# ESMWG/NoahMP

Measured on AMD Instinct MI355X. Metric: column-steps/sec, higher is better.
Workload: dtype f32

## Files before the change

### noahmp_amd/csrc/nmp_dev_column.hpp

```cpp
#pragma once
#ifndef __HIPCC_RTC__
#include <string.h>
#endif
#include "nmp_dev_sflx.hpp"
#include "nmp_dev_glacier.hpp"

namespace nmp {

struct KArgs {
  noahmp_step_args a;
  Ctx c;
  int ni, nka;
  int nti, ntj;
  int k1;
  int kp_lo, kp_hi;
  int yearlen;
  unsigned long long* err;
  int* counts;
  unsigned long long err_base;
  long t_offset;
  long t_first, t_count;
  long r_land, r_ice, r_skip;
};

constexpr int LAY_SLOTS = 4 * NL + 5 * NSOIL + 3 * NSNOW;

template <int STRIDE>
NMP_DEV Lay<LArr<STRIDE>> make_lay(float* base) {
  Lay<LArr<STRIDE>> y;
  int o = 0;
  y.stc.p = base + o * STRIDE; o += NL;
  y.zsnso.p = base + o * STRIDE; o += NL;
  y.dzsnso.p = base + o * STRIDE; o += NL;
  y.imelt.p = base + o * STRIDE; o += NL;
  y.smc.p = base + (o - L(1)) * STRIDE; o += NSOIL;
  y.sh2o.p = base + (o - L(1)) * STRIDE; o += NSOIL;
  y.sice.p = base + (o - L(1)) * STRIDE; o += NSOIL;
  y.smceq.p = base + (o - L(1)) * STRIDE; o += NSOIL;
  y.btrani.p = base + (o - L(1)) * STRIDE; o += NSOIL;
  y.snice.p = base + o * STRIDE; o += NSNOW;
  y.snliq.p = base + o * STRIDE; o += NSNOW;
  y.ficeold.p = base + o * STRIDE; o += NSNOW;
  return y;
}

#ifdef NMP_WIDE_INDEX
typedef size_t nmp_ij_t;
#define G2(f) k.a.f[ij]
#define G3(f, lev, nk) k.a.f[((size_t)jj * (nk) + (lev)) * k.ni + ii]
#else
typedef uint32_t nmp_ij_t;
template <class T> NMP_DEV T& at32(T* base, uint32_t idx) {
  const uint32_t o = idx * (uint32_t)sizeof(T);
  return *(T*)((char*)base + (size_t)o);
}
#define G2(f) nmp::at32(k.a.f, ij)
#define G3(f, lev, nk) nmp::at32(k.a.f, ((uint32_t)jj * (uint32_t)(nk) + (uint32_t)(lev)) * (uint32_t)k.ni + (uint32_t)ii)
#endif


NMP_DEV bool column_index(const KArgs& k, long t, int& ii, int& jj, nmp_ij_t& ij) {
  if (t >= (long)k.nti * k.ntj) return false;
  const int tj = (int)(t / k.nti), ti = (int)(t - (long)tj * k.nti);
  ii = k.a.its - k.a.ims + ti;
  jj = k.a.jts - k.a.jms + tj;
  ij = (nmp_ij_t)jj * (nmp_ij_t)k.ni + (nmp_ij_t)ii;
  return true;
}

NMP_DEV int column_classify_values(const KArgs& k, float xland, float xice, int ivg, int ii, int jj, nmp_ij_t ij) {
  int ice = (xice >= k.a.xice_thres) ? 1 : ((ivg == k.a.isice) ? -1 : 0);
  const bool water = (xland - 1.5f) >= 0.f;
  if (k.a.itimestep == 1) {
    if (water) {
      G2(smstav) = 1.0f; G2(smstot) = 1.0f;
      for (int l = 0; l < NSOIL; l++) { G3(smois, l, NSOIL) = 1.0f; G3(tslb, l, NSOIL) = 273.16f; }
    } else if (xice == 1.f) {
      G2(smstav) = 1.0f; G2(smstot) = 1.0f;
      for (int l = 0; l < NSOIL; l++) G3(smois, l, NSOIL) = 1.0f;
    }
  }
  if (water) return 2;
  if (ice == 1) {
    for (int l = 0; l < NSOIL; l++) G3(sh2o, l, NSOIL) = 1.0f;
    G2(xlaixy) = 0.01f;
    return 2;
  }
  return (ice == -1) ? 1 : 0;
}

NMP_DEV int column_classify(const KArgs& k, long t, int& ii, int& jj, nmp_ij_t& ij) {
  if (!column_index(k, t, ii, jj, ij)) return 3;
  const float xland = G2(xland), xice = G2(xice);
  const int ivg = G2(ivgtyp);
  return column_classify_values(k, xland, xice, ivg, ii, jj, ij);
}

NMP_DEV void scatter_energy_outputs(const KArgs& k, const Col& s, nmp_ij_t ij) {
  G2(tsk) = s.trad; G2(hfx) = s.fsh; G2(grdflx) = s.ssoil;
  if (s.albedo > -999) G2(albedo) = s.albedo;
  G2(snowc) = s.fsno; G2(emiss) = s.emissi;
  G2(tgxy) = s.tg; G2(eahxy) = s.eah; G2(tahxy) = s.tah; G2(cmxy) = s.cm; G2(chxy) = s.ch;
  G2(alboldxy) = s.albold; G2(taussxy) = s.tauss; G2(sneqvoxy) = s.sneqvo;
  G2(t2mvxy) = s.t2mv; G2(t2mbxy) = s.t2mb; G2(q2mvxy) = s.q2v / (1.0f - s.q2v);
  G2(tradxy) = s.trad; G2(fvegxy) = s.fveg; G2(fsaxy) = s.fsa; G2(firaxy) = s.fira;
  G2(aparxy) = s.apar; G2(psnxy) = s.psn; G2(savxy) = s.sav; G2(sagxy) = s.sag;
  G2(rssunxy) = s.rssun; G2(rsshaxy) = s.rssha; G2(bgapxy) = s.bgap; G2(wgapxy) = s.wgap;
  G2(tgvxy) = s.tgv; G2(tgbxy) = s.tgb; G2(chvxy) = s.chv; G2(chbxy) = s.chb;
  G2(ircxy) = s.irc; G2(irgxy) = s.irg; G2(shcxy) = s.shc; G2(shgxy) = s.shg; G2(evgxy) = s.evg;
  G2(ghvxy) = s.ghv; G2(irbxy) = s.irb; G2(shbxy) = s.shb; G2(evbxy) = s.evb; G2(ghbxy) = s.ghb;
  G2(trxy) = s.tr; G2(evcxy) = s.evc; G2(chleafxy) = s.chleaf; G2(chucxy) = s.chuc;
  G2(chv2xy) = s.chv2; G2(chb2xy) = s.chb2;
}

NMP_DEV void gather_water_state(const KArgs& k, Col& s, nmp_ij_t ij) {
  s.wslake = G2(wslakexy); s.zwt = G2(zwtxy); s.wt = G2(wtxy);
  s.lfmass = G2(lfmassxy); s.rtmass = G2(rtmassxy); s.stmass = G2(stmassxy); s.wood = G2(woodxy);
  s.stblcp = G2(stblcpxy); s.fastcp = G2(fastcpxy);
  s.smcwtd = G2(smcwtdxy);
  s.acc_sfcrunoff = G2(sfcrunoff); s.acc_udrunoff = G2(udrunoff); s.acc_acsnow = G2(acsnow); s.acc_acsnom = G2(acsnom);
  s.acc_rech = G2(rechxy); s.acc_deeprech = G2(deeprechxy);
}

template <int STRIDE, int MODE = 0, bool EARLY = false, class Runner>
NMP_DEV int column_step(const KArgs& k, int cls, int ii, int jj, nmp_ij_t ij, float* base, Runner& runner, int* cls_out = nullptr) {
  Lay<LArr<STRIDE>> y = make_lay<STRIDE>(base);
  Col s = {};
  Parm P = {};
  bool live = (cls == 0);
  int failed = 0;
  int soiltyp_w = 1;
  NMP_TIC0();
  float c_xland = 0.f, c_xice = 0.f;
  int c_ivg = 0;
  if (EARLY) { c_xland = G2(xland); c_xice = G2(xice); c_ivg = G2(ivgtyp); }
  if (EARLY || cls <= 1) {
  int vegtyp = EARLY ? c_ivg : G2(ivgtyp), soiltyp = G2(isltyp);
  const float xice_in = EARLY ? c_xice : G2(xice);
  s.lat = G2(xlatin);
  s.cosz = G2(coszin);
  const float dz8w_in = G3(dz8w, k.k1, k.nka), vegfra_in = G2(vegfra), vegmax_in = G2(vegmax);
  s.tbot = G2(tmn);
  s.sfctmp = G3(t3d, k.k1, k.nka);
  const float qv_in = G3(qv3d, k.k1, k.nka);
  s.uu = G3(u_phy, k.k1, k.nka); s.vv = G3(v_phy, k.k1, k.nka);
  s.soldn = G2(swdown); s.lwdn = G2(glw);
  const float p8w_hi = G3(p8w3d, k.kp_hi, k.nka), p8w_lo = G3(p8w3d, k.kp_lo, k.nka);
  s.psfc = G3(p8w3d, k.k1, k.nka);
  const float rainbl_in = G2(rainbl);
  int isnow_in = G2(isnowxy);
  float smc_in[NSOIL], sh2o_in[NSOIL], tslb_in[NSOIL], smceq_in[NSOIL], tsno_in[3], snice_in[3], snliq_in[3], zsnso_in[NL];
#pragma unroll
  for (int l = 1; l <= NSOIL; l++) {
    smc_in[l - 1] = G3(smois, l - 1, NSOIL); sh2o_in[l - 1] = G3(sh2o, l - 1, NSOIL);
    tslb_in[l - 1] = G3(tslb, l - 1, NSOIL); smceq_in[l - 1] = G3(smoiseq, l - 1, NSOIL);
  }
#pragma unroll
  for (int l = -2; l <= 0; l++) {
    snice_in[l + 2] = G3(snicexy, l + 2, 3); snliq_in[l + 2] = G3(snliqxy, l + 2, 3); tsno_in[l + 2] = G3(tsnoxy, l + 2, 3);
  }
#pragma unroll
  for (int l = -2; l <= NSOIL; l++) zsnso_in[L(l)] = G3(zsnsoxy, l + 2, NSOIL + 3);
  s.sneqv = G2(snow); s.snowh = G2(snowh); s.qsfc = G2(qsfc);
  s.tv = G2(tvxy); s.tg = G2(tgxy); s.canliq = G2(canliqxy); s.canice = G2(canicexy);
  s.eah = G2(eahxy); s.tah = G2(tahxy); s.cm = G2(cmxy); s.ch = G2(chxy); s.fwet = G2(fwetxy);
  s.sneqvo = G2(sneqvoxy); s.albold = G2(alboldxy); s.qsnow = G2(qsnowxy);
  s.lai = G2(xlaixy); s.sai = G2(xsaixy);
  s.tauss = G2(taussxy); s.wa = G2(waxy);
  if (EARLY) {
    cls = column_classify_values(k, c_xland, c_xice, c_ivg, ii, jj, ij);
    if (cls_out) *cls_out = cls;
    if (cls != MODE - 1) return 0;
    live = (cls == 0);
  }
  s.ist = 1; s.isc = 4; s.ice = (cls == 1) ? -1 : 0;
  s.yearlen = k.yearlen; s.julian = k.a.julian;
  if (isnow_in < -NSNOW || isnow_in > 0) raise(s, NOAHMP_ERR_ISNOW_RANGE);
  s.isnow = isnow_in < -NSNOW ? -NSNOW : (isnow_in > 0 ? 0 : isnow_in);
  NMP_ASSUME(s.isnow >= -NSNOW && s.isnow <= 0);
  if (soiltyp == 14 && xice_in == 0.f) soiltyp = 7;
  if (vegtyp == k.a.isurban || vegtyp == 31 || vegtyp == 32 || vegtyp == 33) vegtyp = k.a.isurban;
  NMP_TIC(0);
  redprm(k.c, s, P, vegtyp, soiltyp);
  soiltyp_w = soiltyp;
  NMP_TIC(1);
  s.zlvl = 0.5f * dz8w_in;
  s.shdfac = div_rc(vegfra_in, NMP_RCC(100.f));
  s.shdmax = div_rc(vegmax_in, NMP_RCC(100.f));
  s.q2 = qv_in / (1.0f + qv_in);
  s.sfcprs = (p8w_hi + p8w_lo) * 0.5f;
  s.prcp = div_rc(rainbl_in, k.c.u.dt);
#pragma unroll
  for (int l = 1; l <= NSOIL; l++) {
    y.smc[L(l)] = smc_in[l - 1]; y.sh2o[L(l)] = sh2o_in[l - 1];
    y.stc[L(l)] = tslb_in[l - 1]; y.smceq[L(l)] = smceq_in[l - 1];
    y.sice[L(l)] = 0.f; y.btrani[L(l)] = 0.f;
  }
#pragma unroll
  for (int l = -2; l <= 0; l++) {
    y.stc[L(l)] = tsno_in[l + 2]; y.snice[L(l)] = snice_in[l + 2]; y.snliq[L(l)] = snliq_in[l + 2];
    y.ficeold[L(l)] = (l > s.isnow) ? snice_in[l + 2] / (snice_in[l + 2] + snliq_in[l + 2]) : 0.f;
  }
#pragma unroll
  for (int l = -2; l <= NSOIL; l++) { y.zsnso[L(l)] = zsnso_in[L(l)]; y.dzsnso[L(l)] = 0.f; y.imelt[L(l)] = 0.f; }
  s.rech = 0.f; s.deeprech = 0.f;
  s.co2air = 395.e-06f * s.sfcprs;
  s.o2air = 0.209f * s.sfcprs;
  s.foln = 1.0f;
  if (vegtyp == 25 || vegtyp == 26 || vegtyp == 27) { s.shdfac = 0.0f; s.lai = 0.0f; }
  s.vegtyp = (vegtyp >= 1 && vegtyp <= k.c.ts.lucats) ? vegtyp : 1;
  if (s.err) { failed = s.err; live = false; }
  }

  float qfx_out = 0.f, lh_out = 0.f;
  if constexpr (MODE != 1)
  if (cls == 1 && !failed) {
    s.tbot = nmp_min(s.tbot, 263.15f);
    glacier(k.c, s, y);
    if (s.err) failed = s.err;
    else {
      gather_water_state(k, s, ij);
      glacier_fill_undefined(s);
      qfx_out = s.edir; lh_out = s.fgev;
      scatter_energy_outputs(k, s, ij);
    }
  }
  if constexpr (MODE != 2) {
    float beg_wb = 0.f;
    bool water_inputs = false;
    auto prefetch_water = [&]() {
      gather_water_state(k, s, ij);
      redprm_water(k.c, P, soiltyp_w, s.vegtyp);
      water_inputs = true;
    };
    sflx_energy(k.c, P, s, y, beg_wb, live, runner, prefetch_water);
    if (live) {
      if (s.err) failed = s.err;
      else {
        lh_out = s.fcev + s.fgev + s.fctr;
        scatter_energy_outputs(k, s, ij);
        if (!water_inputs) prefetch_water();
        NMP_TIC(11);
        sflx_water(k.c, P, s, y, beg_wb);
        if (s.err) failed = s.err;
        qfx_out = s.ecan + s.edir + s.etran;
      }
    }
  }
  if (cls > 1 || failed) return failed;
  G2(qfx) = qfx_out; G2(lh) = lh_out;
  G2(smstav) = 0.0f; G2(smstot) = 0.0f;
  G2(sfcrunoff) = s.acc_sfcrunoff + s.runsrf * k.a.dt;
  G2(udrunoff) = s.acc_udrunoff + s.runsub * k.a.dt;
#pragma unroll
  for (int l = 1; l <= NSOIL; l++) {
    G3(smois, l - 1, NSOIL) = y.smc[L(l)]; G3(sh2o, l - 1, NSOIL) = y.sh2o[L(l)];
    G3(tslb, l - 1, NSOIL) = y.stc[L(l)];
  }
  G2(snow) = s.sneqv; G2(snowh) = s.snowh;
  G2(canwat) = s.canliq + s.canice;
  G2(acsnow) = s.acc_acsnow + s.prcp * s.fpice;
  G2(acsnom) = s.acc_acsnom + s.qsnbot * k.a.dt + s.ponding + s.ponding1 + s.ponding2;
  G2(qsfc) = s.qsfc;
  G2(isnowxy) = s.isnow; G2(tvxy) = s.tv; G2(canliqxy) = s.canliq; G2(canicexy) = s.canice;
  G2(fwetxy) = s.fwet; G2(qsnowxy) = s.qsnow;
  G2(wslakexy) = s.wslake; G2(zwtxy) = s.zwt; G2(waxy) = s.wa; G2(wtxy) = s.wt;
#pragma unroll
  for (int l = -2; l <= 0; l++) {
    G3(tsnoxy, l + 2, 3) = y.stc[L(l)]; G3(snicexy, l + 2, 3) = y.snice[L(l)];
    G3(snliqxy, l + 2, 3) = y.snliq[L(l)];
  }
#pragma unroll
  for (int l = -2; l <= NSOIL; l++) G3(zsnsoxy, l + 2, NSOIL + 3) = y.zsnso[L(l)];
  G2(lfmassxy) = s.lfmass; G2(rtmassxy) = s.rtmass; G2(stmassxy) = s.stmass; G2(woodxy) = s.wood;
  G2(stblcpxy) = s.stblcp; G2(fastcpxy) = s.fastcp; G2(xlaixy) = s.lai; G2(xsaixy) = s.sai;
  G2(q2mbxy) = s.q2b / (1.0f - s.q2b);
  G2(neexy) = s.nee; G2(gppxy) = s.gpp; G2(nppxy) = s.npp;
  G2(runsfxy) = s.runsrf; G2(runsbxy) = s.runsub; G2(ecanxy) = s.ecan;
  G2(edirxy) = s.edir; G2(etranxy) = s.etran;
  G2(rechxy) = s.acc_rech + s.rech * 1.E3f;
  G2(deeprechxy) = s.acc_deeprech + s.deeprech;
  G2(smcwtdxy) = s.smcwtd;
  NMP_TIC(15);
  return 0;
}

}
```

### noahmp_amd/csrc/nmp_kernel.hpp

```cpp
#pragma once
#ifndef __HIPCC_RTC__
#include <hip/hip_runtime.h>
#endif
#include "nmp_dev_column.hpp"
#ifndef __HIPCC_RTC__
#include "nmp_engine_host.hpp"
#else
namespace nmp_host { constexpr int kCountSlots = 256, kCountStride = 16; }
#endif

namespace {
using namespace nmp;

#ifndef NMP_WAVES_PER_EU
#define NMP_WAVES_PER_EU 2
#endif
#ifndef NMP_FIXED_BLOCK
#define NMP_FIXED_BLOCK 64
#endif

template <int BLOCK, bool USE_LDS, int MODE>
__device__ __forceinline__ void column_kernel_body(const KArgs& k, float* lds, const long blk, const long first, const long count) {
  constexpr int STRIDE = USE_LDS ? BLOCK : 1;
  float priv[(USE_LDS || MODE == 3) ? 1 : LAY_SLOTS];
  float* base = USE_LDS ? (lds + threadIdx.x) : priv;

  if (MODE != 3) libm::libm_stage_tables();
  const long tl = blk * BLOCK + threadIdx.x;
  const long t = first + tl;
  int ii = 0, jj = 0;
  nmp_ij_t ij = 0;
  int cls = 3, err = 0;
  if (MODE == 1 || MODE == 2) {
    if (tl < count && column_index(k, t, ii, jj, ij)) {
      SimpleLoop runner;
      err = column_step<STRIDE, MODE, true>(k, -1, ii, jj, ij, base, runner, &cls);
    }
  } else {
    cls = (MODE != 0 && tl >= count) ? 3 : column_classify(k, t, ii, jj, ij);
  }
  {
    unsigned long long m0 = __ballot(cls == 0), m1 = __ballot(cls == 1), m2 = __ballot(cls == 2);
    if ((threadIdx.x & 63) == 0) {
      int* cnt = k.counts + (blockIdx.x % nmp_host::kCountSlots) * nmp_host::kCountStride;
      if (m0) atomicAdd(&cnt[0], __popcll(m0));
      if (m1) atomicAdd(&cnt[1], __popcll(m1));
      if (m2) atomicAdd(&cnt[2], __popcll(m2));
    }
  }
  if (MODE != 0 && cls != 3 && cls != MODE - 1) {
    atomicMin(k.err, k.err_base | ((unsigned long long)(t + k.t_offset + 1) << 8) | (unsigned)NOAHMP_ERR_CLASS_RANGE);
    return;
  }
  if (MODE == 1 || MODE == 2) {
    if (err) atomicMin(k.err, k.err_base | ((unsigned long long)(t + k.t_offset + 1) << 8) | (unsigned)err);
    return;
  }
  if (cls > 1 || MODE == 3) return;
  SimpleLoop runner;
  err = column_step<STRIDE, (MODE == 3 ? 0 : MODE)>(k, cls, ii, jj, ij, base, runner);
  if (err) atomicMin(k.err, k.err_base | ((unsigned long long)(t + k.t_offset + 1) << 8) | (unsigned)err);
}

template <int BLOCK, bool USE_LDS, int MODE = 0>
__global__ void __launch_bounds__(BLOCK, NMP_WAVES_PER_EU) noahmp_column_kernel(const KArgs k) {
  __shared__ float lds[(USE_LDS && MODE != 3) ? LAY_SLOTS * BLOCK : 1];
  column_kernel_body<BLOCK, USE_LDS, MODE>(k, lds, (long)blockIdx.x, k.t_first, k.t_count);
}

template <int BLOCK>
__global__ void __launch_bounds__(BLOCK, NMP_WAVES_PER_EU) noahmp_ranges_kernel(const KArgs k) {
  __shared__ float lds[LAY_SLOTS * BLOCK];
  const long nb_ice = (k.r_ice + BLOCK - 1) / BLOCK, nb_land = (k.r_land + BLOCK - 1) / BLOCK;
  const long b = (long)blockIdx.x;
  if (b < nb_ice) column_kernel_body<BLOCK, true, 2>(k, lds, b, k.r_land, k.r_ice);
  else if (b < nb_ice + nb_land) column_kernel_body<BLOCK, true, 1>(k, lds, b - nb_ice, 0L, k.r_land);
  else column_kernel_body<BLOCK, true, 3>(k, lds, b - nb_ice - nb_land, k.r_land + k.r_ice, k.r_skip);
}

}
```

### noahmp_amd/csrc/nmp_libm.hpp

```cpp
#pragma once
#ifndef __HIPCC_RTC__
#include <hip/hip_runtime.h>
#include <stdint.h>
#include <string.h>
#endif

namespace nmp {
namespace libm {

#ifndef NMP_LIBM_DEV
#define NMP_LIBM_DEV __host__ __device__ __forceinline__
#endif
#ifndef NMP_LIBM_FN
#define NMP_LIBM_FN NMP_LIBM_DEV
#endif
#ifndef NMP_LIBM_FN_POW
#define NMP_LIBM_FN_POW NMP_LIBM_FN
#endif

#if defined(__HIP_DEVICE_COMPILE__)
#define NMP_LIBM_TABLE static __device__ const
#else
#define NMP_LIBM_TABLE static const
#endif
#include "nmp_libm_tables.inc"
#ifndef NMP_LIBM_LDS
#define NMP_LIBM_LDS 1
#endif
#if defined(__HIP_DEVICE_COMPILE__) && NMP_LIBM_LDS
static __shared__ uint64_t sExp2fTab[32];
static __shared__ double sLogfTab[32];
static __shared__ double sPowfLog2Tab[32];
#define NMP_T_EXP2F sExp2fTab
#define NMP_T_LOGF sLogfTab
#define NMP_T_POWLOG2 sPowfLog2Tab
__device__ __forceinline__ void libm_stage_tables() {
  const int t = threadIdx.y * blockDim.x + threadIdx.x;
  if (t < 32) {
    sExp2fTab[t] = kExp2fTab[t];
    sLogfTab[t] = kLogfTab[t];
    sPowfLog2Tab[t] = kPowfLog2Tab[t];
  }
  __syncthreads();
}
#else
#define NMP_T_EXP2F kExp2fTab
#define NMP_T_LOGF kLogfTab
#define NMP_T_POWLOG2 kPowfLog2Tab
__host__ __device__ __forceinline__ void libm_stage_tables() {}
#endif

NMP_LIBM_DEV double mad(double a, double b, double c) { return __builtin_fma(a, b, c); }

NMP_LIBM_DEV uint32_t asuint(float f) { uint32_t u; memcpy(&u, &f, 4); return u; }
NMP_LIBM_DEV float asfloat(uint32_t u) { float f; memcpy(&f, &u, 4); return f; }
NMP_LIBM_DEV uint64_t asuint64(double f) { uint64_t u; memcpy(&u, &f, 8); return u; }
NMP_LIBM_DEV double asdouble(uint64_t u) { double f; memcpy(&f, &u, 8); return f; }
NMP_LIBM_DEV uint64_t exp2_tab_scale_(uint64_t tab, uint64_t k) {
#if defined(__HIP_DEVICE_COMPILE__)
  if (!__builtin_constant_p(k)) {
    typedef uint32_t u32x2 __attribute__((ext_vector_type(2)));
    u32x2 w = __builtin_bit_cast(u32x2, tab);
    w.y += (uint32_t)k << (52 - 5 - 32);
    return __builtin_bit_cast(uint64_t, w);
  }
#endif
  return tab + (k << (52 - 5));
}

NMP_LIBM_DEV bool expf_is_special_(float x) { return !(__builtin_fabsf(x) <= 88.0f); }
NMP_LIBM_DEV float expf_special_(float x, float res) {
  res = (x > 0x1.62e42ep6f) ? asfloat(0x7f800000u) : res;
  res = (x < -0x1.9fe368p6f) ? 0.0f : res;
  res = (x != x) ? x + x : res;
  return res;
}
NMP_LIBM_FN float expf_(float x) {
  const double xd = (double)x;
  double z = kExpfInvLn2Scaled * xd;
  double kd = z + kExp2fShift;
  const uint64_t ki = asuint64(kd);
  kd -= kExp2fShift;
  const double r = mad(kExpfInvLn2Scaled, xd, -kd);
  const uint64_t t = exp2_tab_scale_(NMP_T_EXP2F[ki % 32], ki);
  const double s = asdouble(t);
  z = mad(kExp2fPolyScaled[0], r, kExp2fPolyScaled[1]);
  const double r2 = r * r;
  double y = mad(kExp2fPolyScaled[2], r, 1.0);
  y = mad(z, r2, y);
  y = y * s;
  float res = (float)y;
  if (__builtin_expect(expf_is_special_(x), 0)) res = expf_special_(x, res);
  return res;
}

NMP_LIBM_DEV float expf_k_(float x) {
  const double xd = (double)x;
  double z = kExpfInvLn2Scaled * xd;
  double kd = z + kExp2fShift;
  const uint64_t ki = asuint64(kd);
  kd -= kExp2fShift;
  const double r = mad(kExpfInvLn2Scaled, xd, -kd);
  const uint64_t t = exp2_tab_scale_(kExp2fTab[ki % 32], ki);
  const double s = asdouble(t);
  z = mad(kExp2fPolyScaled[0], r, kExp2fPolyScaled[1]);
  const double r2 = r * r;
  double y = mad(kExp2fPolyScaled[2], r, 1.0);
  y = mad(z, r2, y);
  y = y * s;
  float res = (float)y;
  res = (x > 0x1.62e42ep6f) ? asfloat(0x7f800000u) : res;
  res = (x < -0x1.9fe368p6f) ? 0.0f : res;
  res = (x != x) ? x + x : res;
  return res;
}

NMP_LIBM_DEV bool logf_is_special_(uint32_t ix) { return ix - 0x00800000u >= 0x7f800000u - 0x00800000u; }
NMP_LIBM_DEV uint32_t logf_normalise_(float x, uint32_t ix) {
  return (ix - 1u < 0x007fffffu) ? asuint(x * 0x1p23f) - (23u << 23) : ix;
}
NMP_LIBM_DEV float logf_fix_special_(uint32_t ix0, float x, float res) {
  res = (ix0 == 0x7f800000u) ? x : res;
  res = ((ix0 & 0x80000000u) || ix0 * 2 > 0xff000000u) ? asfloat(0x7fc00000u) : res;
  res = (ix0 * 2 == 0) ? -asfloat(0x7f800000u) : res;
  return res;
}
NMP_LIBM_FN float logf_(float x) {
  const uint32_t ix0 = asuint(x);
  uint32_t ix = ix0;
  if (__builtin_expect(logf_is_special_(ix0), 0)) ix = logf_normalise_(x, ix0);
  const uint32_t tmp = ix - 0x3f330000u;
  const int i = (tmp >> (23 - 4)) % 16;
  const int k = (int32_t)tmp >> 23;
  const uint32_t iz = ix - (tmp & 0xff800000u);
  const double invc = NMP_T_LOGF[2 * i], logc = NMP_T_LOGF[2 * i + 1];
  const double z = (double)asfloat(iz);
  const double r = mad(z, invc, -1.0);
  const double y0 = mad((double)k, kLogfLn2, logc);
  const double r2 = r * r;
  double y = mad(kLogfPoly[1], r, kLogfPoly[2]);
  y = mad(kLogfPoly[0], r2, y);
  y = mad(y, r2, y0 + r);
  float res = (float)y;
  if (__builtin_expect(logf_is_special_(ix0), 0)) res = logf_fix_special_(ix0, x, res);
  return res;
}

#if defined(__HIP_DEVICE_COMPILE__)
#define NMP_LIBM_PIN() __builtin_amdgcn_sched_barrier(0)
#else
#define NMP_LIBM_PIN() ((void)0)
#endif
template <int N>
NMP_LIBM_DEV void logfN_(const float* x, float* out) {
  uint32_t ix0[N], ixn[N], iz[N]; int k[N]; double invc[N], logc[N];
  bool special = false;
#pragma unroll
  for (int n = 0; n < N; n++) {
    ix0[n] = asuint(x[n]);
    ixn[n] = ix0[n];
    special = special || logf_is_special_(ix0[n]);
  }
  if (__builtin_expect(special, 0)) {
#pragma unroll
    for (int n = 0; n < N; n++) ixn[n] = logf_normalise_(x[n], ix0[n]);
  }
#pragma unroll
  for (int n = 0; n < N; n++) {
    const uint32_t ix = ixn[n];
    const uint32_t tmp = ix - 0x3f330000u;
    const int i = (tmp >> (23 - 4)) % 16;
    k[n] = (int32_t)tmp >> 23;
    iz[n] = ix - (tmp & 0xff800000u);
    invc[n] = NMP_T_LOGF[2 * i]; logc[n] = NMP_T_LOGF[2 * i + 1];
  }
  NMP_LIBM_PIN();
#pragma unroll
  for (int n = 0; n < N; n++) {
    const double z = (double)asfloat(iz[n]);
    const double r = mad(z, invc[n], -1.0);
    const double y0 = mad((double)k[n], kLogfLn2, logc[n]);
    const double r2 = r * r;
    double y = mad(kLogfPoly[1], r, kLogfPoly[2]);
    y = mad(kLogfPoly[0], r2, y);
    y = mad(y, r2, y0 + r);
    out[n] = (float)y;
  }
  if (__builtin_expect(special, 0)) {
#pragma unroll
    for (int n = 0; n < N; n++) out[n] = logf_fix_special_(ix0[n], x[n], out[n]);
  }
}
template <int N>
NMP_LIBM_DEV void expfN_(const float* x, float* out) {
  double r[N]; uint64_t t[N];
#pragma unroll
  for (int n = 0; n < N; n++) {
    const double xd = (double)x[n];
    const double z = kExpfInvLn2Scaled * xd;
    double kd = z + kExp2fShift;
    const uint64_t ki = asuint64(kd);
    kd -= kExp2fShift;
// ... 592 lines not shown
```

### noahmp_amd/csrc/noahmp_engine.hip

```cpp
#include <hip/hip_runtime.h>
#include <stdio.h>
#include <stdlib.h>
#include <string.h>
#include <string>
#include <vector>
#include "noahmp_hip.h"
#define NMP_WIDE_INDEX 1
#include "nmp_kernel.hpp"
#include "nmp_stage.hpp"

using namespace nmp;

namespace {

struct FieldDesc { const char* name; size_t off; int kind; int lev; int io; };
#define FD(n, kind, lev, io) {#n, offsetof(noahmp_step_args, n), kind, lev, io}
const FieldDesc kFields[] = {
#include "nmp_fields.inc"
};
constexpr int kNumFields = sizeof(kFields) / sizeof(kFields[0]);

}

namespace nmp_host {
// ... 100 lines not shown
  if (rc) return rc;
  if (!bytes) return 0;
  if (kind == 2) { HIPCHK(hipMemcpy(dst, src, bytes, hipMemcpyDeviceToDevice)); return 0; }
  rc = kind == 0 ? nmp_host::copy_h2d(dst, src, bytes, g.own_stream) : nmp_host::copy_d2h(dst, src, bytes, g.own_stream);
  if (rc) return rc;
  HIPCHK(hipStreamSynchronize(g.own_stream));
  return 0;
}
void noahmp_hip_free(void* p) { if (p) hipFree(p); }

static void drop_host_regs();

int noahmp_hip_debug_live_host_registrations(void) {
  int n = 0;
  for (auto& kv : g.host_regs) n += kv.second.state == 1;
  return n;
}

int noahmp_hip_set_tables(const noahmp_tables* t) {
  int rc = ensure_init();
  if (rc) return rc;
  drop_host_regs();
  g.out_mirror_valid = false;
  static nmp::TablesDev img;
  img.t = *t;
  nmp::derive_tables(img.t, img.d);
  if (!g.d_tables) HIPCHK(hipMalloc((void**)&g.d_tables, sizeof(nmp::TablesDev)));
  HIPCHK(hipMemcpy(g.d_tables, &img, sizeof(nmp::TablesDev), hipMemcpyHostToDevice));
  nmp::tab_scalars_pack(nmp::tab_scalars(img.t), g.ts_i, g.ts_f);
  g.have_tables = true;
  return 0;
}

static void note_fetch(int rc) {
  if (rc > 0) {
    g.deferred_code = rc;
    g.last_error = std::string("a fatal column of the previous (deferred) step is pending: ") + noahmp_hip_error_string(rc);
  }
}

int noahmp_hip_set_option(const char* key, int value) {
  int prev = -1;
  if (!strcmp(key, "block")) { prev = g.block; if (value == 64 || value == 128 || value == 256) g.block = value; }
  else if (!strcmp(key, "lds")) { prev = g.use_lds; g.use_lds = value ? 1 : 0; }
  else if (!strcmp(key, "host_chunks")) {
    prev = g.host_chunks_auto ? -2 : g.host_chunks;
    if (value == -1 || value == -2) g.host_chunks_auto = true;
    else if (value >= 0 && value <= 32) { g.host_chunks = value; g.host_chunks_auto = false; }
  }
  else if (!strcmp(key, "pin_host_arrays")) {
    prev = g.pin_host_arrays;
    if (value == 0 || value == 1) {
      g.pin_host_arrays = value;
      if (!value) drop_host_regs();
    }
  }
  else if (!strcmp(key, "trust_out_mirror")) {
    prev = g.trust_out_mirror;
    if (value == 0 || value == 1) { g.trust_out_mirror = value; g.out_mirror_valid = false; }
  }
  else if (!strcmp(key, "jit_option_kernels")) { prev = g.jit_kernels; if (value == 0 || value == 1) g.jit_kernels = value; }
  else if (!strcmp(key, "jit_compile_only")) { prev = g.jit_compile_only; if (value == 0 || value == 1) g.jit_compile_only = value; }
  else if (!strcmp(key, "fixed_option_kernels")) { prev = g.fixed_kernels; if (value == 0 || value == 1) g.fixed_kernels = value; }
  else if (!strcmp(key, "sorted_land_columns")) { prev = (int)g.sorted_land; g.sorted_land = value; }
  else if (!strcmp(key, "sorted_glacier_columns")) { prev = (int)g.sorted_glacier; g.sorted_glacier = value; }
  else if (!strcmp(key, "resident_state")) {
    prev = g.resident_state;
    if (value == 0 || value == 1) {
      if (!value && (g.resident_dirty || g.deferred_pending)) note_fetch(noahmp_hip_fetch(nullptr));
      g.resident_state = value; g.resident_valid = false;
    }
  }
  else if (!strcmp(key, "resident_sorted")) {
    prev = g.resident_sorted;
    if (value == 0 || value == 1) {
      if (value != g.resident_sorted && (g.resident_dirty || g.deferred_pending)) note_fetch(noahmp_hip_fetch(nullptr));
      if (value != g.resident_sorted) { g.resident_sorted = value; g.sorted_ok = false; g.resident_valid = false; }
    }
  }
  else if (!strcmp(key, "lazy_download")) {
    prev = g.lazy_download;
    if (value == 0 || value == 1) {
      if (!value && (g.resident_dirty || g.deferred_pending)) note_fetch(noahmp_hip_fetch(nullptr));
      g.lazy_download = value;
    }
  }
  else if (!strcmp(key, "overlap_class_kernels")) prev = 1;
  else if (!strcmp(key, "static_inputs")) {
    prev = g.static_inputs;
    if ((value == 0 || value == 1) && value != g.static_inputs) {
      if (g.resident_dirty || g.deferred_pending) note_fetch(noahmp_hip_fetch(nullptr));
      g.static_inputs = value; g.sorted_ok = false; g.sorted_newer = false; g.resident_valid = false;
    }
  }
  else if (!strcmp(key, "deferred_status")) {
    prev = g.deferred_status;
    if (value == 0 || value == 1) {
      if (g.deferred_pending || g.resident_dirty) note_fetch(noahmp_hip_fetch(nullptr));
      g.deferred_status = value; g.resident_valid = false;
    }
  }
  else if (!strcmp(key, "record_cost")) {
#ifdef NMP_COST_RECORD
    prev = g.record_cost;
    if (value == 0 || value == 1) { g.record_cost = value; if (!value) g.cost_fresh = false; }
#endif
  }
  else if (!strcmp(key, "exact_libm")) prev = NMP_EXACT_LIBM;
  return prev;
}

}

static void fill_kargs(KArgs& k, const noahmp_step_args* a) {
  memset(&k, 0, sizeof(k));
  k.a = *a;
  k.ni = a->ime - a->ims + 1;
  k.nka = a->kme - a->kms + 1;
  k.nti = a->ite - a->its + 1;
  k.ntj = a->jte - a->jts + 1;
  k.k1 = 1 - a->kms;
  k.kp_lo = a->kts - a->kms;
  k.kp_hi = a->kts + 1 - a->kms;
  k.yearlen = 365;
  if (a->yr % 4 == 0) { k.yearlen = 366; if (a->yr % 100 == 0) { k.yearlen = 365; if (a->yr % 400 == 0) k.yearlen = 366; } }
  k.c.T = g.d_tables;
  k.c.D = derived_of(g.d_tables);
  k.c.O = Opt{a->idveg, a->iopt_crs, a->iopt_btr, a->iopt_run, a->iopt_sfc, a->iopt_frz, a->iopt_inf,
              a->iopt_rad, a->iopt_alb, a->iopt_snf, a->iopt_tbot, a->iopt_stc};
  k.c.dt = a->dt;
  k.c.isurban = a->isurban;
  k.c.ts = tab_scalars_unpack(g.ts_i, g.ts_f);
  k.c.zsoil[L(1)] = -a->dzs[0];
  for (int l = 2; l <= NOAHMP_NSOIL; l++) k.c.zsoil[L(l)] = -a->dzs[l - 1] + k.c.zsoil[L(l - 1)];
  ctx_fill_uniform(k.c);
  k.err = g.d_err;
  k.counts = g.d_counts;
  k.a.dzs = nullptr;
}

#ifndef NMP_NO_FIXED_KERNELS
struct FixedKernel { int dveg, run; void (*launch)(const nmp_host::LaunchDesc&, int, hipStream_t, hipEvent_t, hipEvent_t); };
static const FixedKernel kFixed[] = {{1, 1, nmp_host::launch_fixed_d1_r1}, {3, 1, nmp_host::launch_fixed_d3_r1},
                                     {3, 5, nmp_host::launch_fixed_d3_r5}, {4, 1, nmp_host::launch_fixed_d4_r1},
                                     {4, 3, nmp_host::launch_fixed_d4_r3}};
#endif
static int fixed_level(const KArgs& k) {
#ifdef NMP_NO_FIXED_KERNELS
  return 0;
#else
  const Opt& o = k.c.O;
  if (!g.fixed_kernels) return 0;
  if (noahmp_hip_index_width(k.ni, k.a.jme - k.a.jms + 1, k.nka) != 32) return 0;
  if (!(o.crs == 1 && o.btr == 1 && o.sfc == 1 && o.frz == 1 && o.inf == 1 && o.rad == 3 && o.alb == 2 &&
        o.snf == 1 && o.tbot == 2 && o.stc == 1)) return g.jit_kernels ? -1 : 0;
  for (int n = 0; n < (int)(sizeof(kFixed) / sizeof(kFixed[0])); n++)
    if (kFixed[n].dveg == o.dveg && kFixed[n].run == o.run) return n + 1;
  return g.jit_kernels ? -1 : 0;
#endif
}

static bool launch_fixed(const KArgs& k, int level, int mode, hipStream_t s, hipEvent_t ev0 = nullptr, hipEvent_t ev1 = nullptr) {
#ifdef NMP_NO_FIXED_KERNELS
  return false;
#else
  nmp_host::LaunchDesc d;
  memset(&d, 0, sizeof(d));
  d.a = k.a; d.tables = k.c.T; d.dt = k.c.dt; d.isurban = k.c.isurban;
  for (int n = 0; n < 6; n++) d.ts_i[n] = g.ts_i[n];
  for (int n = 0; n < 15; n++) d.ts_f[n] = g.ts_f[n];
  for (int l = 0; l < NL; l++) d.zsoil[l] = k.c.zsoil[l];
  d.ni = k.ni; d.nka = k.nka; d.nti = k.nti; d.ntj = k.ntj; d.k1 = k.k1; d.kp_lo = k.kp_lo; d.kp_hi = k.kp_hi; d.yearlen = k.yearlen;
  d.err = k.err; d.counts = k.counts; d.err_base = k.err_base; d.t_offset = k.t_offset; d.t_first = k.t_first; d.t_count = k.t_count;
  d.cost = k.c.cost;
  d.r_land = k.r_land; d.r_ice = k.r_ice; d.r_skip = k.r_skip;
  if (level > 0) { kFixed[level - 1].launch(d, mode, s, ev0, ev1); return true; }
  const Opt& o = k.c.O;
  const int opts[12] = {o.dveg, o.crs, o.btr, o.run, o.sfc, o.frz, o.inf, o.rad, o.alb, o.snf, o.tbot, o.stc};
  return nmp_host::launch_jit(opts, d, mode, s, ev0, ev1);
#endif
}

static void launch_ranges(KArgs k, long n_land, long n_ice, long n_skip, hipStream_t s, hipEvent_t ev0, hipEvent_t ev1) {
  constexpr long B = NMP_FIXED_BLOCK;
  k.r_land = n_land; k.r_ice = n_ice; k.r_skip = n_skip;
  k.t_first = 0; k.t_count = n_land + n_ice + n_skip;
  const long nb_ice = (n_ice + B - 1) / B, nb = nb_ice + (n_land + B - 1) / B + (n_skip + B - 1) / B;
  if (nb <= 0) return;
  if (k.c.cost) k.c.cost -= 2 * nb_ice * B;
  const int fx = fixed_level(k);
  if (fx && launch_fixed(k, fx, 4, s, ev0, ev1)) return;
  hipExtLaunchKernelGGL((noahmp_ranges_kernel<NMP_FIXED_BLOCK>), dim3((unsigned)nb), dim3(NMP_FIXED_BLOCK), 0, s, ev0, ev1, 0, k);
}

static void launch_any(const KArgs& k_in, hipStream_t s, bool class_ranges = false, hipEvent_t* ev = nullptr) {
  KArgs k = k_in;
  const long ncol = (long)k.nti * k.ntj;
  g.last_launch_kind = 0;
  if (ncol <= 0) { g.last_launch_kind = -1; return; }
  k.c.cost = nullptr;
  if (g.record_cost && class_ranges && k.t_offset == 0) {
    if (nmp_host::ensure_bytes((void**)&g.d_cost, &g.d_cost_bytes, (size_t)ncol * 2) == 0) {
      if (g.cost_cols != ncol) (void)hipMemsetAsync(g.d_cost, 0, (size_t)ncol * 2, s);
      k.c.cost = g.d_cost; g.cost_cols = ncol; g.cost_fresh = true;
    }
  }
  if (class_ranges && g.sorted_land >= 0 && g.sorted_glacier >= 0 && g.sorted_land + g.sorted_glacier <= ncol && k.t_offset == 0 &&
      g.block == 256 && g.use_lds) {
    g.last_launch_kind = 1;
    launch_ranges(k, g.sorted_land, g.sorted_glacier, ncol - g.sorted_land - g.sorted_glacier, s, ev ? ev[0] : nullptr, ev ? ev[1] : nullptr);
    return;
  }
  if (ev) hipEventRecord(ev[0], s);
  struct EndEvent { hipEvent_t* e; hipStream_t s; ~EndEvent() { if (e) hipEventRecord(e[1], s); } } at_end{ev, s};
  if (g.block == 256 && g.use_lds) {
    const int fx = fixed_level(k);
    if (fx) { k.t_first = 0; k.t_count = ncol; if (launch_fixed(k, fx, 0, s)) return; }
  }
  if (g.block == 256) launch<256>(k, ncol, g.use_lds, s);
  else if (g.block == 128) launch<128>(k, ncol, g.use_lds, s);
  else launch<64>(k, ncol, g.use_lds, s);
}

static int check_step_args(const noahmp_step_args* a, noahmp_status* st) {
  if (!g.have_tables) { g.last_error = "noahmp_hip_set_tables() has not been called"; return -102; }
  if (a->nsoil != NOAHMP_NSOIL) { if (st) st->code = NOAHMP_ERR_NSOIL_UNSUPPORTED; return NOAHMP_ERR_NSOIL_UNSUPPORTED; }
  if (a->iopt_sfc != 1 && a->iopt_sfc != 2) {
    if (st) st->code = NOAHMP_ERR_OPT_SFC_UNSUPPORTED;
    return NOAHMP_ERR_OPT_SFC_UNSUPPORTED;
  }
  return 0;
}

static void drop_host_regs() {
  bool any = false;
  for (auto& kv : g.host_regs) any = any || kv.second.state == 1;
  if (any) hipDeviceSynchronize();
  for (auto& kv : g.host_regs) if (kv.second.state == 1) hipHostUnregister(const_cast<void*>(kv.first));
  g.host_regs.clear();
  (void)hipGetLastError();
}
static void maybe_pin(const void* host, size_t bytes) {
  if (!g.pin_host_arrays || !host || !bytes) return;
  const char* lo = (const char*)host; const char* hi = lo + bytes;
  for (auto it = g.host_regs.begin(); it != g.host_regs.end();) {
    const char* olo = (const char*)it->first; const char* ohi = olo + it->second.bytes;
    if (it->first != host && olo < hi && lo < ohi) {
      if (it->second.state == 1) { hipDeviceSynchronize(); hipHostUnregister(const_cast<void*>(it->first)); }
      it = g.host_regs.erase(it);
    } else ++it;
  }
  auto it = g.host_regs.find(host);
  if (it == g.host_regs.end()) { g.host_regs[host] = nmp_host::Engine::HostReg{bytes, 1, 0}; (void)hipGetLastError(); return; }
  nmp_host::Engine::HostReg& r = it->second;
  if (r.bytes != bytes) {
    if (r.state == 1) { hipDeviceSynchronize(); hipHostUnregister(const_cast<void*>(host)); }
    r = nmp_host::Engine::HostReg{bytes, 1, 0};
    (void)hipGetLastError();
    return;
  }
  r.seen++;
  if (r.state == 0 && r.seen >= 2)
    r.state = hipHostRegister(const_cast<void*>(host), bytes, hipHostRegisterDefault) == hipSuccess ? 1 : -1;
  (void)hipGetLastError();
}

static int pipeline_chunks(const noahmp_step_args* a) {
  if (!g.host_chunks_auto) return g.host_chunks;
  const long ncol = (long)(a->ite - a->its + 1) * (a->jte - a->jts + 1);
  const long n = (ncol + 600000) / 1200000;
  return (int)(n < 3 ? 3 : (n > 8 ? 8 : n));
}
static int step_host_pipelined(const noahmp_step_args* a, hipStream_t s, noahmp_status* st) {
  KArgs k;
  fill_kargs(k, a);
  const int nj_mem = a->jme - a->jms + 1;
  if (!g.s_up) { HIPCHK(hipStreamCreateWithFlags(&g.s_up, hipStreamNonBlocking)); HIPCHK(hipStreamCreateWithFlags(&g.s_dn, hipStreamNonBlocking)); }
  const int want = pipeline_chunks(a);
  const int nreg = want < nj_mem ? want : nj_mem;
  std::vector<int> rows;
  rows.push_back(0);
  for (int c = 0; c < nreg; c++) {
    const int r0 = (int)((long)nj_mem * c / nreg), r1 = (int)((long)nj_mem * (c + 1) / nreg);
    if (c == 0 && g.host_chunks_auto && r1 - r0 >= 8) rows.push_back(r0 + (r1 - r0) / 4);
    rows.push_back(r1);
  }
  const int nchunk = (int)rows.size() - 1;
  while ((int)g.pipe_events.size() < 3 * nchunk) { hipEvent_t e; HIPCHK(hipEventCreate(&e)); g.pipe_events.push_back(e); }
  if (g.pipe_host.size() != (size_t)kNumFields) { g.pipe_host.assign(kNumFields, nullptr); g.out_mirror_valid = false; }
  {
    const int ext[9] = {a->ims, a->ime, a->jms, a->jme, a->kms, a->kme, a->nsoil, 0, 0};
    if (memcmp(ext, g.pipe_extents, sizeof ext)) { memcpy(g.pipe_extents, ext, sizeof ext); g.out_mirror_valid = false; }
  }
  for (int f = 0; f < kNumFields; f++) {
    const void* host = *(void* const*)((const char*)a + kFields[f].off);
    if (g.pipe_host[f] != host) { g.pipe_host[f] = host; g.out_mirror_valid = false; }
  }
  const bool upload_out = !(g.trust_out_mirror && g.out_mirror_valid);
  size_t rowbytes[kNumFields];
  for (int f = 0; f < kNumFields; f++) {
    const FieldDesc& fd = kFields[f];
    const size_t bytes = field_elems(fd, a) * 4;
    rowbytes[f] = bytes / nj_mem;
    if (g.mirror_bytes[f] < bytes) {
      if (g.mirror[f]) HIPCHK(hipFree(g.mirror[f]));
      HIPCHK(hipMalloc(&g.mirror[f], bytes));
// ... 670 lines not shown
```

Measured before the change: 2.152 billion.

## Split libm table staging, pin output pointers in SGPRs, batch final stores

Result: no change. 2.164 billion (median of 6 runs) (+0.6%).

```diff
diff --git a/noahmp_amd/csrc/nmp_dev_column.hpp b/noahmp_amd/csrc/nmp_dev_column.hpp
--- a/noahmp_amd/csrc/nmp_dev_column.hpp
+++ b/noahmp_amd/csrc/nmp_dev_column.hpp
@@ -59,9 +59,23 @@
 #endif
 
 
+#if defined(__HIP_DEVICE_COMPILE__) && !defined(NMP_NO_PIN_PTRS)
+#define NMP_P(f) "s"(k.a.f)
+#define NMP_PIN_PTRS(...) asm volatile("" :: __VA_ARGS__)
+#define NMP_PIN_PTRS_IF(cond, ...) do { if constexpr (cond) asm volatile("" :: __VA_ARGS__); } while (0)
+#else
+#define NMP_PIN_PTRS(...) ((void)0)
+#define NMP_PIN_PTRS_IF(cond, ...) ((void)0)
+#endif
+
 NMP_DEV bool column_index(const KArgs& k, long t, int& ii, int& jj, nmp_ij_t& ij) {
   if (t >= (long)k.nti * k.ntj) return false;
+#ifdef NMP_WIDE_INDEX
   const int tj = (int)(t / k.nti), ti = (int)(t - (long)tj * k.nti);
+#else
+  const uint32_t tu = (uint32_t)t, tju = tu / (uint32_t)k.nti;
+  const int tj = (int)tju, ti = (int)(tu - tju * (uint32_t)k.nti);
+#endif
   ii = k.a.its - k.a.ims + ti;
   jj = k.a.jts - k.a.jms + tj;
   ij = (nmp_ij_t)jj * (nmp_ij_t)k.ni + (nmp_ij_t)ii;
@@ -96,19 +110,27 @@
   return column_classify_values(k, xland, xice, ivg, ii, jj, ij);
 }
 
-NMP_DEV void scatter_energy_outputs(const KArgs& k, const Col& s, nmp_ij_t ij) {
+template <bool PIN> NMP_DEV void scatter_energy_outputs(const KArgs& k, const Col& s, nmp_ij_t ij) {
+  NMP_PIN_PTRS_IF(PIN, NMP_P(tsk), NMP_P(hfx), NMP_P(grdflx), NMP_P(snowc), NMP_P(emiss), NMP_P(tgxy), NMP_P(eahxy), NMP_P(albedo));
   G2(tsk) = s.trad; G2(hfx) = s.fsh; G2(grdflx) = s.ssoil;
   if (s.albedo > -999) G2(albedo) = s.albedo;
-  G2(snowc) = s.fsno; G2(emiss) = s.emissi;
-  G2(tgxy) = s.tg; G2(eahxy) = s.eah; G2(tahxy) = s.tah; G2(cmxy) = s.cm; G2(chxy) = s.ch;
+  G2(snowc) = s.fsno; G2(emiss) = s.emissi; G2(tgxy) = s.tg; G2(eahxy) = s.eah;
+  NMP_PIN_PTRS_IF(PIN, NMP_P(tahxy), NMP_P(cmxy), NMP_P(chxy), NMP_P(alboldxy), NMP_P(taussxy), NMP_P(sneqvoxy), NMP_P(t2mvxy), NMP_P(t2mbxy));
+  G2(tahxy) = s.tah; G2(cmxy) = s.cm; G2(chxy) = s.ch;
   G2(alboldxy) = s.albold; G2(taussxy) = s.tauss; G2(sneqvoxy) = s.sneqvo;
-  G2(t2mvxy) = s.t2mv; G2(t2mbxy) = s.t2mb; G2(q2mvxy) = s.q2v / (1.0f - s.q2v);
+  G2(t2mvxy) = s.t2mv; G2(t2mbxy) = s.t2mb;
+  NMP_PIN_PTRS_IF(PIN, NMP_P(q2mvxy), NMP_P(tradxy), NMP_P(fvegxy), NMP_P(fsaxy), NMP_P(firaxy), NMP_P(aparxy), NMP_P(psnxy), NMP_P(savxy));
+  G2(q2mvxy) = s.q2v / (1.0f - s.q2v);
   G2(tradxy) = s.trad; G2(fvegxy) = s.fveg; G2(fsaxy) = s.fsa; G2(firaxy) = s.fira;
-  G2(aparxy) = s.apar; G2(psnxy) = s.psn; G2(savxy) = s.sav; G2(sagxy) = s.sag;
-  G2(rssunxy) = s.rssun; G2(rsshaxy) = s.rssha; G2(bgapxy) = s.bgap; G2(wgapxy) = s.wgap;
-  G2(tgvxy) = s.tgv; G2(tgbxy) = s.tgb; G2(chvxy) = s.chv; G2(chbxy) = s.chb;
-  G2(ircxy) = s.irc; G2(irgxy) = s.irg; G2(shcxy) = s.shc; G2(shgxy) = s.shg; G2(evgxy) = s.evg;
-  G2(ghvxy) = s.ghv; G2(irbxy) = s.irb; G2(shbxy) = s.shb; G2(evbxy) = s.evb; G2(ghbxy) = s.ghb;
+  G2(aparxy) = s.apar; G2(psnxy) = s.psn; G2(savxy) = s.sav;
+  NMP_PIN_PTRS_IF(PIN, NMP_P(sagxy), NMP_P(rssunxy), NMP_P(rsshaxy), NMP_P(bgapxy), NMP_P(wgapxy), NMP_P(tgvxy), NMP_P(tgbxy), NMP_P(chvxy));
+  G2(sagxy) = s.sag; G2(rssunxy) = s.rssun; G2(rsshaxy) = s.rssha; G2(bgapxy) = s.bgap; G2(wgapxy) = s.wgap;
+  G2(tgvxy) = s.tgv; G2(tgbxy) = s.tgb; G2(chvxy) = s.chv;
+  NMP_PIN_PTRS_IF(PIN, NMP_P(chbxy), NMP_P(ircxy), NMP_P(irgxy), NMP_P(shcxy), NMP_P(shgxy), NMP_P(evgxy), NMP_P(ghvxy), NMP_P(irbxy));
+  G2(chbxy) = s.chb; G2(ircxy) = s.irc; G2(irgxy) = s.irg; G2(shcxy) = s.shc; G2(shgxy) = s.shg; G2(evgxy) = s.evg;
+  G2(ghvxy) = s.ghv; G2(irbxy) = s.irb;
+  NMP_PIN_PTRS_IF(PIN, NMP_P(shbxy), NMP_P(evbxy), NMP_P(ghbxy), NMP_P(trxy), NMP_P(evcxy), NMP_P(chleafxy), NMP_P(chucxy), NMP_P(chv2xy), NMP_P(chb2xy));
+  G2(shbxy) = s.shb; G2(evbxy) = s.evb; G2(ghbxy) = s.ghb;
   G2(trxy) = s.tr; G2(evcxy) = s.evc; G2(chleafxy) = s.chleaf; G2(chucxy) = s.chuc;
   G2(chv2xy) = s.chv2; G2(chb2xy) = s.chb2;
 }
@@ -123,7 +145,8 @@
 }
 
 template <int STRIDE, int MODE = 0, bool EARLY = false, class Runner>
-NMP_DEV int column_step(const KArgs& k, int cls, int ii, int jj, nmp_ij_t ij, float* base, Runner& runner, int* cls_out = nullptr) {
+NMP_DEV int column_step(const KArgs& k, int cls, int ii, int jj, nmp_ij_t ij, float* base, Runner& runner, int* cls_out = nullptr,
+                        const libm::LibmTables* tabs = nullptr, bool tabs_all = false) {
   Lay<LArr<STRIDE>> y = make_lay<STRIDE>(base);
   Col s = {};
   Parm P = {};
@@ -167,6 +190,9 @@
   s.sneqvo = G2(sneqvoxy); s.albold = G2(alboldxy); s.qsnow = G2(qsnowxy);
   s.lai = G2(xlaixy); s.sai = G2(xsaixy);
   s.tauss = G2(taussxy); s.wa = G2(waxy);
+#if NMP_LIBM_STAGED
+  if (tabs) libm::libm_commit_tables_wave(*tabs, (int)threadIdx.x, tabs_all);
+#endif
   if (EARLY) {
     cls = column_classify_values(k, c_xland, c_xice, c_ivg, ii, jj, ij);
     if (cls_out) *cls_out = cls;
@@ -222,7 +248,7 @@
       gather_water_state(k, s, ij);
       glacier_fill_undefined(s);
       qfx_out = s.edir; lh_out = s.fgev;
-      scatter_energy_outputs(k, s, ij);
+      scatter_energy_outputs<MODE != 0>(k, s, ij);
     }
   }
   if constexpr (MODE != 2) {
@@ -238,7 +264,7 @@
       if (s.err) failed = s.err;
       else {
         lh_out = s.fcev + s.fgev + s.fctr;
-        scatter_energy_outputs(k, s, ij);
+        scatter_energy_outputs<MODE != 0>(k, s, ij);
         if (!water_inputs) prefetch_water();
         NMP_TIC(11);
         sflx_water(k.c, P, s, y, beg_wb);
@@ -248,15 +274,25 @@
     }
   }
   if (cls > 1 || failed) return failed;
+  float smc_out[NSOIL], sh2o_out[NSOIL], stc_out[NL], snice_out[NSNOW], snliq_out[NSNOW], zsnso_out[NL];
+#pragma unroll
+  for (int l = 1; l <= NSOIL; l++) { smc_out[l - 1] = y.smc[L(l)]; sh2o_out[l - 1] = y.sh2o[L(l)]; }
+#pragma unroll
+  for (int l = -2; l <= 0; l++) { snice_out[l + 2] = y.snice[L(l)]; snliq_out[l + 2] = y.snliq[L(l)]; }
+#pragma unroll
+  for (int l = -2; l <= NSOIL; l++) { stc_out[L(l)] = y.stc[L(l)]; zsnso_out[L(l)] = y.zsnso[L(l)]; }
+  NMP_PIN_PTRS(NMP_P(qfx), NMP_P(lh), NMP_P(smstav), NMP_P(smstot), NMP_P(sfcrunoff), NMP_P(udrunoff), NMP_P(smois), NMP_P(sh2o), NMP_P(tslb));
   G2(qfx) = qfx_out; G2(lh) = lh_out;
   G2(smstav) = 0.0f; G2(smstot) = 0.0f;
   G2(sfcrunoff) = s.acc_sfcrunoff + s.runsrf * k.a.dt;
   G2(udrunoff) = s.acc_udrunoff + s.runsub * k.a.dt;
 #pragma unroll
   for (int l = 1; l <= NSOIL; l++) {
-    G3(smois, l - 1, NSOIL) = y.smc[L(l)]; G3(sh2o, l - 1, NSOIL) = y.sh2o[L(l)];
-    G3(tslb, l - 1, NSOIL) = y.stc[L(l)];
-  }
+    G3(smois, l - 1, NSOIL) = smc_out[l - 1]; G3(sh2o, l - 1, NSOIL) = sh2o_out[l - 1];
+    G3(tslb, l - 1, NSOIL) = stc_out[L(l)];
+  }
+  NMP_PIN_PTRS(NMP_P(snow), NMP_P(snowh), NMP_P(canwat), NMP_P(acsnow), NMP_P(acsnom), NMP_P(qsfc), NMP_P(isnowxy), NMP_P(tvxy),
+               NMP_P(canliqxy), NMP_P(canicexy), NMP_P(fwetxy), NMP_P(qsnowxy));
   G2(snow) = s.sneqv; G2(snowh) = s.snowh;
   G2(canwat) = s.canliq + s.canice;
   G2(acsnow) = s.acc_acsnow + s.prcp * s.fpice;
@@ -264,16 +300,20 @@
   G2(qsfc) = s.qsfc;
   G2(isnowxy) = s.isnow; G2(tvxy) = s.tv; G2(canliqxy) = s.canliq; G2(canicexy) = s.canice;
   G2(fwetxy) = s.fwet; G2(qsnowxy) = s.qsnow;
+  NMP_PIN_PTRS(NMP_P(wslakexy), NMP_P(zwtxy), NMP_P(waxy), NMP_P(wtxy), NMP_P(tsnoxy), NMP_P(snicexy), NMP_P(snliqxy), NMP_P(zsnsoxy));
   G2(wslakexy) = s.wslake; G2(zwtxy) = s.zwt; G2(waxy) = s.wa; G2(wtxy) = s.wt;
 #pragma unroll
   for (int l = -2; l <= 0; l++) {
-    G3(tsnoxy, l + 2, 3) = y.stc[L(l)]; G3(snicexy, l + 2, 3) = y.snice[L(l)];
-    G3(snliqxy, l + 2, 3) = y.snliq[L(l)];
-  }
-#pragma unroll
-  for (int l = -2; l <= NSOIL; l++) G3(zsnsoxy, l + 2, NSOIL + 3) = y.zsnso[L(l)];
+    G3(tsnoxy, l + 2, 3) = stc_out[L(l)]; G3(snicexy, l + 2, 3) = snice_out[l + 2];
+    G3(snliqxy, l + 2, 3) = snliq_out[l + 2];
+  }
+#pragma unroll
+  for (int l = -2; l <= NSOIL; l++) G3(zsnsoxy, l + 2, NSOIL + 3) = zsnso_out[L(l)];
+  NMP_PIN_PTRS(NMP_P(lfmassxy), NMP_P(rtmassxy), NMP_P(stmassxy), NMP_P(woodxy), NMP_P(stblcpxy), NMP_P(fastcpxy), NMP_P(xlaixy), NMP_P(xsaixy));
   G2(lfmassxy) = s.lfmass; G2(rtmassxy) = s.rtmass; G2(stmassxy) = s.stmass; G2(woodxy) = s.wood;
   G2(stblcpxy) = s.stblcp; G2(fastcpxy) = s.fastcp; G2(xlaixy) = s.lai; G2(xsaixy) = s.sai;
+  NMP_PIN_PTRS(NMP_P(q2mbxy), NMP_P(neexy), NMP_P(gppxy), NMP_P(nppxy), NMP_P(runsfxy), NMP_P(runsbxy), NMP_P(ecanxy), NMP_P(edirxy),
+               NMP_P(etranxy), NMP_P(rechxy), NMP_P(deeprechxy), NMP_P(smcwtdxy));
   G2(q2mbxy) = s.q2b / (1.0f - s.q2b);
   G2(neexy) = s.nee; G2(gppxy) = s.gpp; G2(nppxy) = s.npp;
   G2(runsfxy) = s.runsrf; G2(runsbxy) = s.runsub; G2(ecanxy) = s.ecan;
diff --git a/noahmp_amd/csrc/nmp_kernel.hpp b/noahmp_amd/csrc/nmp_kernel.hpp
--- a/noahmp_amd/csrc/nmp_kernel.hpp
+++ b/noahmp_amd/csrc/nmp_kernel.hpp
@@ -18,6 +18,9 @@
 #ifndef NMP_FIXED_BLOCK
 #define NMP_FIXED_BLOCK 64
 #endif
+#ifndef NMP_SPLIT_STAGE
+#define NMP_SPLIT_STAGE 1
+#endif
 
 template <int BLOCK, bool USE_LDS, int MODE>
 __device__ __forceinline__ void column_kernel_body(const KArgs& k, float* lds, const long blk, const long first, const long count) {
@@ -25,19 +28,25 @@
   float priv[(USE_LDS || MODE == 3) ? 1 : LAY_SLOTS];
   float* base = USE_LDS ? (lds + threadIdx.x) : priv;
 
-  if (MODE != 3) libm::libm_stage_tables();
+  constexpr bool SPLIT_STAGE = NMP_LIBM_STAGED && NMP_SPLIT_STAGE && BLOCK == 64 && MODE != 3;
+  libm::LibmTables tabs = {};
+  if (SPLIT_STAGE) tabs = libm::libm_fetch_tables((int)threadIdx.x);
+  else if (MODE != 3) libm::libm_stage_tables((int)threadIdx.x);
   const long tl = blk * BLOCK + threadIdx.x;
   const long t = first + tl;
   int ii = 0, jj = 0;
   nmp_ij_t ij = 0;
   int cls = 3, err = 0;
   if (MODE == 1 || MODE == 2) {
-    if (tl < count && column_index(k, t, ii, jj, ij)) {
+    const bool has = tl < count && column_index(k, t, ii, jj, ij);
+    const bool tabs_all = SPLIT_STAGE && (unsigned)__ballot(has) == 0xffffffffu;
+    if (has) {
       SimpleLoop runner;
-      err = column_step<STRIDE, MODE, true>(k, -1, ii, jj, ij, base, runner, &cls);
+      err = column_step<STRIDE, MODE, true>(k, -1, ii, jj, ij, base, runner, &cls, SPLIT_STAGE ? &tabs : nullptr, tabs_all);
     }
   } else {
     cls = (MODE != 0 && tl >= count) ? 3 : column_classify(k, t, ii, jj, ij);
+    if (SPLIT_STAGE) libm::libm_commit_tables(tabs, (int)threadIdx.x);
   }
   {
     unsigned long long m0 = __ballot(cls == 0), m1 = __ballot(cls == 1), m2 = __ballot(cls == 2);
diff --git a/noahmp_amd/csrc/nmp_libm.hpp b/noahmp_amd/csrc/nmp_libm.hpp
--- a/noahmp_amd/csrc/nmp_libm.hpp
+++ b/noahmp_amd/csrc/nmp_libm.hpp
@@ -34,8 +34,7 @@
 #define NMP_T_EXP2F sExp2fTab
 #define NMP_T_LOGF sLogfTab
 #define NMP_T_POWLOG2 sPowfLog2Tab
-__device__ __forceinline__ void libm_stage_tables() {
-  const int t = threadIdx.y * blockDim.x + threadIdx.x;
+__device__ __forceinline__ void libm_stage_tables(int t) {
   if (t < 32) {
     sExp2fTab[t] = kExp2fTab[t];
     sLogfTab[t] = kLogfTab[t];
@@ -43,11 +42,39 @@
   }
   __syncthreads();
 }
+__device__ __forceinline__ void libm_stage_tables() { libm_stage_tables((int)(threadIdx.y * blockDim.x + threadIdx.x)); }
+struct LibmTables { uint64_t e; double l, p; };
+__device__ __forceinline__ LibmTables libm_fetch_tables(int t) {
+  LibmTables r;
+  r.e = kExp2fTab[t & 31]; r.l = kLogfTab[t & 31]; r.p = kPowfLog2Tab[t & 31];
+  return r;
+}
+__device__ __forceinline__ void libm_commit_tables_wave(const LibmTables& r, int t, bool all) {
+  if (all) {
+    sExp2fTab[t & 31] = r.e; sLogfTab[t & 31] = r.l; sPowfLog2Tab[t & 31] = r.p;
+  } else {
+#pragma unroll 1
+    for (int e = 0; e < 32; e++) { sExp2fTab[e] = kExp2fTab[e]; sLogfTab[e] = kLogfTab[e]; sPowfLog2Tab[e] = kPowfLog2Tab[e]; }
+  }
+  __builtin_amdgcn_fence(__ATOMIC_RELEASE, "wavefront");
+  __builtin_amdgcn_fence(__ATOMIC_ACQUIRE, "wavefront");
+}
+__device__ __forceinline__ void libm_commit_tables(const LibmTables& r, int t) {
+  if (t < 32) { sExp2fTab[t] = r.e; sLogfTab[t] = r.l; sPowfLog2Tab[t] = r.p; }
+  __syncthreads();
+}
+#define NMP_LIBM_STAGED 1
 #else
 #define NMP_T_EXP2F kExp2fTab
 #define NMP_T_LOGF kLogfTab
 #define NMP_T_POWLOG2 kPowfLog2Tab
 __host__ __device__ __forceinline__ void libm_stage_tables() {}
+__host__ __device__ __forceinline__ void libm_stage_tables(int) {}
+struct LibmTables {};
+__host__ __device__ __forceinline__ LibmTables libm_fetch_tables(int) { return LibmTables(); }
+__host__ __device__ __forceinline__ void libm_commit_tables_wave(const LibmTables&, int, bool) {}
+__host__ __device__ __forceinline__ void libm_commit_tables(const LibmTables&, int) {}
+#define NMP_LIBM_STAGED 0
 #endif
 
 NMP_LIBM_DEV double mad(double a, double b, double c) { return __builtin_fma(a, b, c); }
diff --git a/noahmp_amd/csrc/noahmp_engine.hip b/noahmp_amd/csrc/noahmp_engine.hip
--- a/noahmp_amd/csrc/noahmp_engine.hip
+++ b/noahmp_amd/csrc/noahmp_engine.hip
@@ -276,6 +276,7 @@
   const Opt& o = k.c.O;
   if (!g.fixed_kernels) return 0;
   if (noahmp_hip_index_width(k.ni, k.a.jme - k.a.jms + 1, k.nka) != 32) return 0;
+  if ((long)k.nti * k.ntj >= (1L << 30)) return 0;
   if (!(o.crs == 1 && o.btr == 1 && o.sfc == 1 && o.frz == 1 && o.inf == 1 && o.rad == 3 && o.alb == 2 &&
         o.snf == 1 && o.tbot == 2 && o.stc == 1)) return g.jit_kernels ? -1 : 0;
   for (int n = 0; n < (int)(sizeof(kFixed) / sizeof(kFixed[0])); n++)
```
